# ivclab/CPG

Measured on AMD Instinct MI355X. Metric: images/sec per CPG train-prune-retrain cycle, VGG16 task-1, higher is better.
Workload: dtype f32; 1 GPU; configs[1]: VGG16-BN custom_vgg 224x224, task-1 CPG cycle (finetune -> prune 0.0->0.1 -> recovery, validate after every 20th train step), batch 256 per GPU; task=1, arch=vgg16, global_batch=256, per_gpu_batch=256, parallelism=dp1, epoch_steps=20

## Files before the change

### cpg_amd/csrc/conv3x3_stem.hip

```cpp
#include <algorithm>
#include <type_traits>
#include "cpg_dispatch.h"

using namespace cpg;

namespace {

typedef float f32x2 __attribute__((ext_vector_type(2)));
constexpr int ST_R = 8, ST_W = 32;
constexpr int ST_PW = 36;
constexpr int ST_ROWS = ST_R + 2;
constexpr int ST_CMAX = 3, ST_KS = 14;
constexpr int ST_PATCH = ST_CMAX * ST_ROWS * ST_PW;

struct StemGeom {
    int N, C, K, H, W;
    int tiles_x, tiles_y;
    unsigned ntiles;
};

enum { ST_PLAIN = 0, ST_STATS = 1, ST_STATS_ONLY = 2, ST_BN_RELU = 3, ST_BWD_REDUCE = 4, ST_BWD_APPLY = 5, ST_BWD_WGRAD = 6 };
constexpr int ST_TS = 36;
struct StemBn {
    const float *gamma, *beta, *mean, *invstd;
    const float *coef;
    const float *gz;
};

template <int MODE, int NB = 2, bool RAG = false>
__global__ __launch_bounds__(256, 2)
void k_stem_fwd(StemGeom g, const float *__restrict__ x, const float *__restrict__ w, const float *__restrict__ pm, float thr,
                const float *__restrict__ bias, float *__restrict__ y, float *__restrict__ stats, StemBn bn) {
    constexpr bool STATS = MODE == ST_STATS || MODE == ST_STATS_ONLY || MODE == ST_BWD_REDUCE;
    constexpr bool BN = MODE >= ST_BN_RELU;
    constexpr bool STORE = MODE == ST_PLAIN || MODE == ST_STATS || MODE == ST_BN_RELU || MODE == ST_BWD_APPLY;
    constexpr bool WG = MODE == ST_BWD_WGRAD;
    constexpr bool TWO_PASS = STATS || BN;
    __shared__ float smem_all[4 * ST_PATCH];
    __shared__ __attribute__((aligned(16))) float cst[(MODE >= ST_BWD_REDUCE) ? NB * 32 * 8 : 4];
    const int tid = threadIdx.x, lane = tid & 63, wave = __builtin_amdgcn_readfirstlane(tid >> 6);
    if constexpr (MODE >= ST_BWD_REDUCE) {
        if (tid < NB * 32) {
            const bool kv = tid < g.K;
            cst[tid * 8 + 0] = kv ? bn.mean[tid] : 0.0f, cst[tid * 8 + 1] = kv ? bn.invstd[tid] : 0.0f;
            cst[tid * 8 + 2] = kv ? bn.gamma[tid] : 0.0f, cst[tid * 8 + 3] = kv ? bn.beta[tid] : 0.0f;
            cst[tid * 8 + 4] = (MODE >= ST_BWD_APPLY && kv) ? bn.coef[2 * tid] : 0.0f;
            cst[tid * 8 + 5] = (MODE >= ST_BWD_APPLY && kv) ? bn.coef[2 * tid + 1] : 0.0f;
        }
        __syncthreads();
    }
    const int li = lane & 31, lh = lane >> 5;
    float *smem = smem_all + wave * ST_PATCH;
    const int HW = g.H * g.W, CK = g.C * 9;
    __shared__ __attribute__((aligned(16))) float tsm_all[WG ? 4 * 32 * ST_TS : 4];
    float *tsm = tsm_all + (WG ? wave * 32 * ST_TS : 0);
    const int wk = li < CK ? li : 0, wboff = ((wk / 9) * ST_ROWS + (wk % 9) / 3) * ST_PW + wk % 3 + lh;
    f32x16 accw[WG ? NB : 1];
    if constexpr (WG) {
#pragma unroll
        for (int mb = 0; mb < NB; ++mb)
#pragma unroll
            for (int e = 0; e < 16; ++e) accw[mb][e] = 0.0f;
    }

    constexpr bool ALDS = NB == 3 && TWO_PASS;
    __shared__ float a_lds[ALDS ? NB * ST_KS * 64 : 1];
    float A[ALDS ? 1 : NB][ST_KS];
    int boff[ST_KS];
#pragma unroll
    for (int t = 0; t < ST_KS; ++t) {
        const int k = 2 * t + lh;
        const bool kv = k < CK;
#pragma unroll
        for (int mb = 0; mb < NB; ++mb) {
            const int co = mb * 32 + li;
            float v = 0.0f;
            if (kv && co < g.K) {
                v = w[co * CK + k];
                if (pm != nullptr) v *= binarize(pm[co * CK + k], thr);
            }
            if constexpr (ALDS) {
                if (wave == 0) a_lds[(mb * ST_KS + t) * 64 + lane] = v;
            } else {
                A[mb][t] = v;
            }
        }
        const int kk = kv ? k : 0;
        const int c = kk / 9, r = (kk % 9) / 3, s = kk % 3;
        boff[t] = (c * ST_ROWS + r) * ST_PW + s + li;
    }
    constexpr bool HASB = !BN;
    constexpr bool BPASS = HASB && TWO_PASS && NB == 3;
    float bv[HASB ? (BPASS ? 1 : NB) : 1][HASB ? 16 : 1];
    if constexpr (HASB && !BPASS) {
#pragma unroll
        for (int mb = 0; mb < NB; ++mb)
#pragma unroll
            for (int e = 0; e < 16; ++e) {
                const int co = mb * 32 + (e & 3) + 8 * (e >> 2) + 4 * lh;
                bv[mb][e] = (bias != nullptr && co < g.K) ? bias[co] : 0.0f;
            }
    }

    const __amdgpu_buffer_rsrc_t srd_x = __builtin_amdgcn_make_buffer_rsrc((void *)x, 0, g.N * g.C * HW * 4, 0x00020000);
    constexpr int kOOR = (int)0x80000000;
    const int hw_half = lane >> 5, hcol = lane & 31;
    float pc[15], ph;
    auto tile_coords = [&](unsigned tile, int &n, int &y0, int &x0) {
        const unsigned per_img = (unsigned)(g.tiles_x * g.tiles_y);
        n = (int)(tile / per_img);
        const unsigned r = tile % per_img;
        y0 = (int)(r / (unsigned)g.tiles_x) * ST_R, x0 = (int)(r % (unsigned)g.tiles_x) * ST_W;
    };
    auto issue_loads = [&](unsigned tile) {
        int n, y0, x0;
        tile_coords(tile, n, y0, x0);
#pragma unroll
        for (int q = 0; q < 15; ++q) {
            const int item = 2 * q + hw_half, c = item / ST_ROWS, r = item % ST_ROWS;
            const int row = y0 - 1 + r, col = x0 + hcol;
            const bool ok = c < g.C && (unsigned)row < (unsigned)g.H && col < g.W;
            const int off = ok ? (((n * g.C + c) * g.H + row) * g.W + col) * 4 : kOOR;
            pc[q] = __builtin_bit_cast(float, __builtin_amdgcn_raw_buffer_load_b32(srd_x, off, 0, 0));
        }
        {
            const int item = lane >> 1, side = lane & 1, c = item / ST_ROWS, r = item % ST_ROWS;
            const int row = y0 - 1 + r, col = side ? x0 + ST_W : x0 - 1;
            const bool ok = item < ST_CMAX * ST_ROWS && c < g.C && (unsigned)row < (unsigned)g.H && (unsigned)col < (unsigned)g.W;
            const int off = ok ? (((n * g.C + c) * g.H + row) * g.W + col) * 4 : kOOR;
            ph = __builtin_bit_cast(float, __builtin_amdgcn_raw_buffer_load_b32(srd_x, off, 0, 0));
        }
    };
    auto write_patch = [&]() {
#pragma unroll
        for (int q = 0; q < 15; ++q) smem[(2 * q + hw_half) * ST_PW + 1 + hcol] = pc[q];
        if (lane < 2 * ST_CMAX * ST_ROWS) smem[(lane >> 1) * ST_PW + ((lane & 1) ? ST_W + 1 : 0)] = ph;
    };

    if constexpr (ALDS) __syncthreads();
    const unsigned nwaves = gridDim.x * 4, wid = blockIdx.x * 4 + wave;
    if (wid >= g.ntiles) return;
    const int HW4 = HW * 4;
    issue_loads(wid);
    for (unsigned tile = wid; tile < g.ntiles; tile += nwaves) {
        int n, y0, x0;
        tile_coords(tile, n, y0, x0);
        write_patch();
        if (tile + nwaves < g.ntiles) issue_loads(tile + nwaves);
        float s1[16], s2[16];
        auto zero_sums = [&]() {
            if (STATS) {
#pragma unroll
                for (int e = 0; e < 16; ++e) s1[e] = s2[e] = 0.0f;
            }
        };
        const __amdgpu_buffer_rsrc_t srd_y = __builtin_amdgcn_make_buffer_rsrc((void *)((STORE ? y : (float *)x) + (STORE ? (int64_t)n * g.K * HW : 0)), 0, STORE ? g.K * HW4 : 0, 0x00020000);
        const __amdgpu_buffer_rsrc_t srd_gz = __builtin_amdgcn_make_buffer_rsrc((void *)(MODE >= ST_BWD_REDUCE ? bn.gz + (int64_t)n * g.K * HW : x), 0, MODE >= ST_BWD_REDUCE ? g.K * HW4 : 0, 0x00020000);
        const bool cok = x0 + li < g.W;
        const int pix0 = (y0 * g.W + x0 + li) * 4 + lh * 4 * HW4;
        const bool full = x0 + ST_W <= g.W && y0 + ST_R <= g.H;
        constexpr bool REGC = MODE == ST_BN_RELU;
        float cm[REGC ? 16 : 1], cis[REGC ? 16 : 1], cga[REGC ? 16 : 1], cbe[REGC ? 16 : 1];
        __amdgpu_buffer_rsrc_t srd_bn[4];
        if constexpr (RAG && REGC) {
            srd_bn[0] = __builtin_amdgcn_make_buffer_rsrc((void *)bn.beta, 0, g.K * 4, 0x00020000);
            srd_bn[1] = __builtin_amdgcn_make_buffer_rsrc((void *)bn.mean, 0, g.K * 4, 0x00020000);
            srd_bn[2] = __builtin_amdgcn_make_buffer_rsrc((void *)bn.invstd, 0, g.K * 4, 0x00020000);
            srd_bn[3] = __builtin_amdgcn_make_buffer_rsrc((void *)bn.gamma, 0, g.K * 4, 0x00020000);
        }
        auto load_bn = [&](int mb) {
            if constexpr (BPASS) {
#pragma unroll
                for (int e = 0; e < 16; ++e) {
                    const int co = mb * 32 + (e & 3) + 8 * (e >> 2) + 4 * lh;
                    bv[0][e] = (bias != nullptr && co < g.K) ? bias[co] : 0.0f;
                }
            }
            if constexpr (ALDS) {
#pragma unroll
                for (int t = 0; t < ST_KS; ++t) A[0][t] = a_lds[(mb * ST_KS + t) * 64 + lane];
            }
            if constexpr (REGC) {
#pragma unroll
                for (int e = 0; e < 16; ++e) {
                    if constexpr (RAG) {
                        const int vo = (4 * lh + (e & 3) + 8 * (e >> 2)) * 4 + mb * 128;
                        cm[e] = __builtin_bit_cast(float, __builtin_amdgcn_raw_buffer_load_b32(srd_bn[1], vo, 0, 0));
                        cis[e] = __builtin_bit_cast(float, __builtin_amdgcn_raw_buffer_load_b32(srd_bn[2], vo, 0, 0));
                        cga[e] = __builtin_bit_cast(float, __builtin_amdgcn_raw_buffer_load_b32(srd_bn[3], vo, 0, 0));
                        cbe[e] = __builtin_bit_cast(float, __builtin_amdgcn_raw_buffer_load_b32(srd_bn[0], vo, 0, 0));
                    } else {
                        const int co = mb * 32 + (e & 3) + 8 * (e >> 2) + 4 * lh;
                        cm[e] = bn.mean[co], cis[e] = bn.invstd[co], cga[e] = bn.gamma[co], cbe[e] = bn.beta[co];
                    }
                }
            }
        };
        auto row = [&](int j, auto fullc, auto mbsel) {
            constexpr bool FULL = decltype(fullc)::value;
            constexpr int MB0 = decltype(mbsel)::value < 0 ? 0 : decltype(mbsel)::value, MB1 = decltype(mbsel)::value < 0 ? NB : MB0 + 1;
            const bool pok = FULL || (cok && y0 + j < g.H);
            const int voff = pok ? pix0 + j * g.W * 4 : kOOR;
            int klim = g.K;
            if constexpr (RAG) asm volatile("" : "+s"(klim));
            auto voff_of = [&](int mb, int e) -> int {
                if constexpr (RAG) {
                    if (mb == NB - 1) return ((NB - 1) * 32 + (e & 3) + 8 * (e >> 2) + 4 * lh < klim) ? voff : kOOR;
                }
                return voff;
            };
            float gzv[MODE >= ST_BWD_REDUCE ? 16 : 1];
            int copq = 0;
            if constexpr (MODE >= ST_BWD_REDUCE) asm volatile("" : "+v"(copq));
            if constexpr (MODE >= ST_BWD_REDUCE) {
#pragma unroll
                for (int e = 0; e < 16; ++e)
                    gzv[e] = __builtin_bit_cast(float, __builtin_amdgcn_raw_buffer_load_b32(srd_gz, voff_of(MB0, e), (MB0 * 32 + (e & 3) + 8 * (e >> 2)) * HW4, 0));
            }
            f32x16 acc[NB];
#pragma unroll
            for (int mb = MB0; mb < MB1; ++mb)
#pragma unroll
                for (int e = 0; e < 16; ++e) acc[mb][e] = 0.0f;
            const float *prow = smem + j * ST_PW;
#pragma unroll
            for (int t = 0; t < ST_KS; ++t) {
                const float b = prow[boff[t]];
#pragma unroll
                for (int mb = MB0; mb < MB1; ++mb) acc[mb] = __builtin_amdgcn_mfma_f32_32x32x2f32(A[ALDS ? 0 : mb][t], b, acc[mb], 0, 0, 0);
            }
#pragma unroll
            for (int mb = MB0; mb < MB1; ++mb)
#pragma unroll
                for (int e = 0; e < 16; ++e) {
                    const int cu = mb * 32 + (e & 3) + 8 * (e >> 2);
                    const float v = HASB ? acc[mb][e] + bv[(HASB && !BPASS) ? mb : 0][HASB ? e : 0] : acc[mb][e];
                    if constexpr (MODE == ST_PLAIN || MODE == ST_STATS) {
                        __builtin_amdgcn_raw_buffer_store_b32(__builtin_bit_cast(int, v), srd_y, voff_of(mb, e), cu * HW4, 0);
                    }
                    if constexpr (MODE == ST_STATS || MODE == ST_STATS_ONLY) {
                        const float vm = (FULL || pok) ? v : 0.0f;
                        s1[e] += vm;
                        s2[e] = fmaf(vm, vm, s2[e]);
                    }
                    if constexpr (MODE == ST_BN_RELU) {
                        const float z = relu_keep((v - cm[e]) * cis[e] * cga[e] + cbe[e]);
                        __builtin_amdgcn_raw_buffer_store_b32(__builtin_bit_cast(int, z), srd_y, voff_of(mb, e), cu * HW4, 0);
                    }
                    if constexpr (MODE >= ST_BWD_REDUCE) {
                        const float *cc = cst + (cu + 4 * lh) * 8 + copq;
                        const f32x4 c4 = *reinterpret_cast<const f32x4 *>(cc);
                        const float xh = (v - c4[0]) * c4[1];
                        const float gm = ((v - c4[0]) * c4[1] * c4[2] + c4[3] > 0.0f) ? gzv[e] : 0.0f;
                        if constexpr (MODE == ST_BWD_REDUCE) {
                            s1[e] += gm;
                            s2[e] = fmaf(gm, xh, s2[e]);
                        } else {
                            const f32x2 c2 = *reinterpret_cast<const f32x2 *>(cc + 4);
                            float gyv = (gm - c2[0] - xh * c2[1]) * (c4[1] * c4[2]);
                            if constexpr (MODE == ST_BWD_APPLY) {
                                __builtin_amdgcn_raw_buffer_store_b32(__builtin_bit_cast(int, gyv), srd_y, voff_of(mb, e), cu * HW4, 0);
                            } else {
                                if (!FULL && !pok) gyv = 0.0f;
                                tsm[((e & 3) + 8 * (e >> 2) + 4 * lh) * ST_TS + (li & 1) * 16 + (li >> 1)] = gyv;
                            }
                        }
                    }
                }
            if constexpr (WG) {
                f32x4 ga[4];
#pragma unroll
                for (int q = 0; q < 4; ++q) ga[q] = *reinterpret_cast<const f32x4 *>(tsm + li * ST_TS + lh * 16 + 4 * q);
                const float *brow = smem + j * ST_PW + wboff;
#pragma unroll
                for (int t = 0; t < 16; ++t)
                    accw[MB0] = __builtin_amdgcn_mfma_f32_32x32x2f32(ga[t >> 2][t & 3], brow[2 * t], accw[MB0], 0, 0, 0);
            }
        };
        auto rows = [&](auto mbsel) {
            if (full) {
#pragma unroll 1
                for (int j = 0; j < ST_R; ++j) row(j, std::true_type{}, mbsel);
            } else {
#pragma unroll 1
                for (int j = 0; j < ST_R; ++j) row(j, std::false_type{}, mbsel);
            }
        };
        auto stats_out = [&](int mb) {
#pragma unroll
            for (int e = 0; e < 16; e += 8) half_wave_sum8(s1 + e), half_wave_sum8(s2 + e);
            if (li == kHalfSumLane) {
#pragma unroll
                for (int e = 0; e < 16; ++e) {
                    const int co = mb * 32 + (e & 3) + 8 * (e >> 2) + 4 * lh;
                    if (RAG && co >= g.K) continue;
                    f32x2 o;
                    o[0] = s1[e], o[1] = s2[e];
                    *reinterpret_cast<f32x2 *>(stats + ((int64_t)co * g.ntiles + tile) * 2) = o;
                }
            }
        };
        if (TWO_PASS) {
            load_bn(0);
            zero_sums();
            rows(std::integral_constant<int, 0>{});
            if (STATS) stats_out(0);
            load_bn(1);
            zero_sums();
            rows(std::integral_constant<int, 1>{});
            if (STATS) stats_out(1);
            if constexpr (NB == 3) {
                load_bn(2);
                zero_sums();
                rows(std::integral_constant<int, 2>{});
                if (STATS) stats_out(2);
            }
        } else {
            rows(std::integral_constant<int, -1>{});
        }
    }
    if constexpr (WG) {
        float *dstw = y + (int64_t)wid * g.K * CK;
#pragma unroll
        for (int mb = 0; mb < NB; ++mb)
#pragma unroll
            for (int e = 0; e < 16; ++e) {
                const int co = mb * 32 + (e & 3) + 8 * (e >> 2) + 4 * lh;
                if (li < CK && co < g.K) dstw[co * CK + li] = accw[mb][e];
            }
    }
}

#define STEM_LAUNCH(MODE, grid, block, shm, stream, ...)                                                          \
    do {                                                                                                          \
        if (g.K == 64) hipLaunchKernelGGL((k_stem_fwd<MODE, 2, false>), grid, block, shm, stream, __VA_ARGS__);   \
        else hipLaunchKernelGGL((k_stem_fwd<MODE, 3, true>), grid, block, shm, stream, __VA_ARGS__);              \
    } while (0)

bool stem_geom(int N, int C, int K, int H, int W, StemGeom &g) {
    if (opt_on(OPT_NO_STEM)) return false;
    if (N < 1 || C < 1 || C > ST_CMAX || K < 64 || K > 96 || H < 1 || W < 1) return false;
    if ((int64_t)N * C * H * W * 4 >= (1ll << 31) || (int64_t)K * H * W * 4 >= (1ll << 31)) return false;
    g.N = N, g.C = C, g.K = K, g.H = H, g.W = W;
    g.tiles_x = (W + ST_W - 1) / ST_W, g.tiles_y = (H + ST_R - 1) / ST_R;
    const int64_t nt = (int64_t)N * g.tiles_x * g.tiles_y;
    if (nt >= (1ll << 31)) return false;
    g.ntiles = (unsigned)nt;
    return true;
}

}

extern "C" int cpg_conv3x3_stem_ok(int N, int C, int K, int H, int W) {
    StemGeom g;
    return stem_geom(N, C, K, H, W, g) ? 1 : 0;
}

extern "C" int cpg_conv3x3_stem_tiles(int N, int C, int K, int H, int W) {
    StemGeom g;
    return stem_geom(N, C, K, H, W, g) ? (int)g.ntiles : 0;
}

extern "C" int cpg_conv3x3_stem_run(int N, int C, int K, int H, int W, const float *x, const float *w, const float *pm, float thr,
                                    const float *bias, float *y, float *stats, hipStream_t stream) {
    StemGeom g;
    if (!stem_geom(N, C, K, H, W, g)) return fail(CPG_E_UNSUPPORTED, "cpg_conv2d_fwd(stem): shape not supported");
    unsigned blocks = (unsigned)std::min<int64_t>(((int64_t)g.ntiles + 3) / 4, 4 * kCUs);
    blocks = (unsigned)std::max(1, opt_or(OPT_STEM_BLOCKS, (int)blocks));
    if (stats != nullptr)
        STEM_LAUNCH(ST_STATS, dim3(blocks), dim3(256), 0, stream, g, x, w, pm, thr, bias, y, stats, StemBn{});
    else
        STEM_LAUNCH(ST_PLAIN, dim3(blocks), dim3(256), 0, stream, g, x, w, pm, thr, bias, y, nullptr, StemBn{});
    CPG_CHECK_LAUNCH("cpg_conv2d_fwd(stem)");
    return CPG_OK;
}

namespace {
bool stem_bn_geom(const cpg_conv_desc *d, StemGeom &g) {
    if (opt_on(OPT_NO_STEM_FUSE)) return false;
    if (!(d->R == 3 && d->S == 3 && d->stride_h == 1 && d->stride_w == 1 && d->pad_h == 1 && d->pad_w == 1 && d->dil_h == 1 &&
          d->dil_w == 1 && d->groups == 1))
        return false;
    return stem_geom(d->N, d->C, d->K, d->H, d->W, g);
}
unsigned stem_blocks(const StemGeom &g) {
    unsigned blocks = (unsigned)std::min<int64_t>(((int64_t)g.ntiles + 3) / 4, 4 * kCUs);
    blocks = (unsigned)std::max(1, opt_or(OPT_STEM_BLOCKS, (int)blocks));
    return blocks;
}
}

extern "C" int32_t cpg_stem_bn_supported(const cpg_conv_desc *d) {
    StemGeom g;
    return (d != nullptr && stem_bn_geom(d, g)) ? 1 : 0;
}
extern "C" int32_t cpg_stem_bn_tiles(const cpg_conv_desc *d) {
    StemGeom g;
    return (d != nullptr && stem_bn_geom(d, g)) ? (int32_t)g.ntiles : 0;
}
extern "C" int cpg_stem_bn_stats(const cpg_conv_desc *d, const float *x, const float *w, const float *pm, float thr, const float *bias,
                                 float *stats, size_t stats_bytes, void *stream_v) {
    StemGeom g;
    CPG_REQUIRE(d && x && w && stats, "cpg_stem_bn_stats: null pointer");
    if (!stem_bn_geom(d, g)) return fail(CPG_E_UNSUPPORTED, "cpg_stem_bn_stats: shape not supported");
    if (bias != nullptr) return fail(CPG_E_UNSUPPORTED, "cpg_stem_bn_stats: the fused stem takes no conv bias");
    if (stats_bytes < (size_t)g.K * g.ntiles * 2 * sizeof(float)) return fail(CPG_E_WORKSPACE, "cpg_stem_bn_stats: statistics buffer too small");
    STEM_LAUNCH(ST_STATS_ONLY, dim3(stem_blocks(g)), dim3(256), 0, (hipStream_t)stream_v, g, x, w, pm, thr, bias,
                       (float *)nullptr, stats, StemBn{});
    CPG_CHECK_LAUNCH("cpg_stem_bn_stats");
    return CPG_OK;
}
extern "C" int cpg_stem_bn_relu_fwd(const cpg_conv_desc *d, const float *x, const float *w, const float *pm, float thr, const float *bias,
                                    const float *gamma, const float *beta, const float *mean, const float *invstd, float *z, void *stream_v) {
    StemGeom g;
    CPG_REQUIRE(d && x && w && gamma && beta && mean && invstd && z, "cpg_stem_bn_relu_fwd: null pointer");
    if (!stem_bn_geom(d, g)) return fail(CPG_E_UNSUPPORTED, "cpg_stem_bn_relu_fwd: shape not supported");
    if (bias != nullptr) return fail(CPG_E_UNSUPPORTED, "cpg_stem_bn_relu_fwd: the fused stem takes no conv bias");
    STEM_LAUNCH(ST_BN_RELU, dim3(stem_blocks(g)), dim3(256), 0, (hipStream_t)stream_v, g, x, w, pm, thr, bias, z,
                       (float *)nullptr, StemBn{gamma, beta, mean, invstd, nullptr, nullptr});
    CPG_CHECK_LAUNCH("cpg_stem_bn_relu_fwd");
    return CPG_OK;
}
extern "C" int cpg_stem_bn_relu_bwd_reduce(const cpg_conv_desc *d, const float *x, const float *w, const float *pm, float thr,
                                           const float *bias, const float *gamma, const float *beta, const float *mean, const float *invstd,
                                           const float *gz, float *partials, size_t partials_bytes, void *stream_v) {
    StemGeom g;
    CPG_REQUIRE(d && x && w && gamma && beta && mean && invstd && gz && partials, "cpg_stem_bn_relu_bwd_reduce: null pointer");
    if (!stem_bn_geom(d, g)) return fail(CPG_E_UNSUPPORTED, "cpg_stem_bn_relu_bwd_reduce: shape not supported");
    if (bias != nullptr) return fail(CPG_E_UNSUPPORTED, "cpg_stem_bn_relu_bwd_reduce: the fused stem takes no conv bias");
    if (partials_bytes < (size_t)g.K * g.ntiles * 2 * sizeof(float)) return fail(CPG_E_WORKSPACE, "cpg_stem_bn_relu_bwd_reduce: partial-sum buffer too small");
    STEM_LAUNCH(ST_BWD_REDUCE, dim3(stem_blocks(g)), dim3(256), 0, (hipStream_t)stream_v, g, x, w, pm, thr, bias,
                       (float *)nullptr, partials, StemBn{gamma, beta, mean, invstd, nullptr, gz});
    CPG_CHECK_LAUNCH("cpg_stem_bn_relu_bwd_reduce");
    return CPG_OK;
}
extern "C" int cpg_stem_bn_relu_bwd_apply(const cpg_conv_desc *d, const float *x, const float *w, const float *pm, float thr,
                                          const float *bias, const float *gamma, const float *beta, const float *mean, const float *invstd,
                                          const float *coef, const float *gz, float *gy, void *stream_v) {
    StemGeom g;
    CPG_REQUIRE(d && x && w && gamma && beta && mean && invstd && coef && gz && gy, "cpg_stem_bn_relu_bwd_apply: null pointer");
    if (!stem_bn_geom(d, g)) return fail(CPG_E_UNSUPPORTED, "cpg_stem_bn_relu_bwd_apply: shape not supported");
    if (bias != nullptr) return fail(CPG_E_UNSUPPORTED, "cpg_stem_bn_relu_bwd_apply: the fused stem takes no conv bias");
    STEM_LAUNCH(ST_BWD_APPLY, dim3(stem_blocks(g)), dim3(256), 0, (hipStream_t)stream_v, g, x, w, pm, thr, bias, gy,
                       (float *)nullptr, StemBn{gamma, beta, mean, invstd, coef, gz});
    CPG_CHECK_LAUNCH("cpg_stem_bn_relu_bwd_apply");
    return CPG_OK;
}

extern "C" size_t cpg_stem_bn_wgrad_workspace(const cpg_conv_desc *d) {
    StemGeom g;
    if (d == nullptr || !stem_bn_geom(d, g)) return 0;
    return (size_t)stem_blocks(g) * 4 * g.K * g.C * 9 * sizeof(float);
}
extern "C" int cpg_stem_bn_relu_bwd_wgrad(const cpg_conv_desc *d, const float *x, const float *w, const float *pm, float thr,
                                          const float *bias, const float *gamma, const float *beta, const float *mean, const float *invstd,
                                          const float *coef, const float *gz, float *gw, float *gpm, void *ws, size_t ws_bytes,
                                          void *stream_v) {
    StemGeom g;
    CPG_REQUIRE(d && x && w && gamma && beta && mean && invstd && coef && gz && gw && ws, "cpg_stem_bn_relu_bwd_wgrad: null pointer");
    CPG_REQUIRE((pm == nullptr) == (gpm == nullptr), "cpg_stem_bn_relu_bwd_wgrad: piggymask and its gradient come as a pair");
    if (!stem_bn_geom(d, g)) return fail(CPG_E_UNSUPPORTED, "cpg_stem_bn_relu_bwd_wgrad: shape not supported");
    if (bias != nullptr) return fail(CPG_E_UNSUPPORTED, "cpg_stem_bn_relu_bwd_wgrad: the fused stem takes no conv bias");
    const unsigned blocks = stem_blocks(g);
    if (ws_bytes < (size_t)blocks * 4 * g.K * g.C * 9 * sizeof(float)) return fail(CPG_E_WORKSPACE, "cpg_stem_bn_relu_bwd_wgrad: workspace too small");
    hipStream_t stream = (hipStream_t)stream_v;
    STEM_LAUNCH(ST_BWD_WGRAD, dim3(blocks), dim3(256), 0, stream, g, x, w, pm, thr, bias, (float *)ws, (float *)nullptr,
                       StemBn{gamma, beta, mean, invstd, coef, gz});
    const int nsplit = (int)std::min<int64_t>((int64_t)g.ntiles, (int64_t)blocks * 4);
    Epilogue ep{gw, nullptr, BIAS_NONE, 1, 1, pm, w, gpm, thr};
    launch_split_reduce((const float *)ws, nsplit, (int64_t)g.K * g.C * 9, 0, ep, stream);
    CPG_CHECK_LAUNCH("cpg_stem_bn_relu_bwd_wgrad");
    return CPG_OK;
}
```

### cpg_amd/csrc/cpg_common.cpp

```cpp
#include "cpg_common.h"
#include <stdarg.h>
#include <stdlib.h>
#include <string.h>
#include <atomic>

namespace cpg {

static thread_local char g_err[512] = "";

char *err_buf() { return g_err; }

int fail(int code, const char *fmt, ...) {
    va_list ap;
    va_start(ap, fmt);
    vsnprintf(g_err, sizeof(g_err), fmt, ap);
    va_end(ap);
    return code;
}

static thread_local PackCtx g_pack = {};
PackCtx &pack_ctx() { return g_pack; }
static thread_local WgradRider g_rider = {};
WgradRider &wgrad_rider() { return g_rider; }
static thread_local PoolMaxCtx g_pool_max = {};
PoolMaxCtx &pool_max_ctx() { return g_pool_max; }
static thread_local PoolMaxCtx g_bn_pool_max = {};
PoolMaxCtx &bn_pool_max_ctx() { return g_bn_pool_max; }

int take_packed(size_t bytes, const float **pre, const char *what) {
    PackCtx &c = g_pack;
    *pre = nullptr;
    if (!c.armed) return CPG_OK;
    if (c.use == nullptr || c.use_bytes != bytes || (((uintptr_t)c.use) & 15) != 0)
        return fail(CPG_E_INVALID, "%s: the packed operand handed in (%zu bytes) is not the one this launch streams (%zu bytes, 16-byte aligned)",
                    what, c.use_bytes, bytes);
    *pre = c.use;
    c.armed = false;
    return CPG_OK;
}

static std::atomic<int> g_shared_chip{0};
int shared_chip_hint() { return g_shared_chip.load(std::memory_order_relaxed); }

namespace {
enum Kind { BOOL, INT, WINO_KERNEL };
struct OptDef {
    const char *name;
    Kind kind;
};
const OptDef kDefs[OPT_COUNT] = {
    {"CPG_NO_WINO", BOOL},          {"CPG_NO_WINO_WGRAD", BOOL},   {"CPG_NO_WINO_ODD", BOOL},      {"CPG_NO_STEM", BOOL},
    {"CPG_NO_STEM_FUSE", BOOL},     {"CPG_NO_DEAD_SKIP", BOOL},    {"CPG_NO_S2", BOOL},            {"CPG_NO_V14", BOOL},
    {"CPG_DISABLE_CONV3X3", BOOL},  {"CPG_DISABLE_CONV1X1", BOOL}, {"CPG_DISABLE_CONV1X1_WGRAD", BOOL}, {"CPG_DISABLE_PW_GEMM", BOOL},
    {"CPG_C3_FORCE", INT},          {"CPG_C3W_BPC", INT},          {"CPG_W3_PICK", INT},           {"CPG_PWW_BPC", INT},
    {"CPG_STEM_BLOCKS", INT},       {"CPG_WINO_KERNEL", WINO_KERNEL}, {"CPG_WINO_NW", INT},        {"CPG_WINO_PERSIST", INT},
    {"CPG_WINO_GRIDS", INT},        {"CPG_WW_UNITS", INT},         {"CPG_WW_XCD", INT},            {"CPG_PW_TILE", INT},           {"CPG_WG3_SHARE", INT},
    {"CPG_WW_SHARE", INT},          {"CPG_WINO_TAIL", INT},         {"CPG_FC_SMALL", INT},
    {"CPG_NO_WW_RIDER", BOOL},      {"CPG_NO_GROUPED", BOOL},       {"CPG_GROUPED_WIDE_MIN", INT},
    {"CPG_NO_POOL_MAX", BOOL},
};

struct Table {
    std::atomic<int> v[OPT_COUNT];
    Table() {
        for (int i = 0; i < OPT_COUNT; ++i) {
            int val = OPT_UNSET;
            if (const char *f = getenv(kDefs[i].name)) {
                switch (kDefs[i].kind) {
                    case BOOL: val = (f[0] == 0 || (f[0] == '0' && f[1] == 0)) ? 0 : 1; break;
                    case INT: val = atoi(f); break;
                    case WINO_KERNEL: val = f[0] == 'b' ? 0 : f[0] == 'p' ? 2 : f[0] == '6' ? 3 : 1; break;
                }
            }
            v[i].store(val, std::memory_order_relaxed);
        }
    }
};
Table g_opts;

int find_opt(const char *name) {
    if (name == nullptr) return -1;
    for (int i = 0; i < OPT_COUNT; ++i)
        if (strcmp(name, kDefs[i].name) == 0) return i;
    return -1;
}
}

int opt(Opt o) { return g_opts.v[o].load(std::memory_order_relaxed); }

}

extern "C" int cpg_set_shared_chip_hint(int32_t shared) {
    cpg::g_shared_chip.store(shared ? 1 : 0, std::memory_order_relaxed);
    return CPG_OK;
}
extern "C" int32_t cpg_get_shared_chip_hint(void) { return cpg::shared_chip_hint(); }
extern "C" int cpg_set_option(const char *name, int32_t value) {
    const int i = cpg::find_opt(name);
    if (i < 0) return cpg::fail(CPG_E_INVALID, "cpg_set_option: unknown option '%s'", name ? name : "(null)");
    cpg::g_opts.v[i].store(value, std::memory_order_relaxed);
    return CPG_OK;
}
extern "C" int cpg_get_option(const char *name, int32_t *value) {
    const int i = cpg::find_opt(name);
    if (i < 0 || value == nullptr) return cpg::fail(CPG_E_INVALID, "cpg_get_option: unknown option '%s'", name ? name : "(null)");
    *value = cpg::g_opts.v[i].load(std::memory_order_relaxed);
    return CPG_OK;
}
extern "C" int cpg_version(void) { return CPG_ABI_VERSION; }
extern "C" const char *cpg_last_error(void) { return cpg::err_buf(); }
```

### cpg_amd/csrc/cpg_common.h

```cpp
#pragma once
#include <hip/hip_runtime.h>
#include <stdint.h>
#include <stdio.h>
#include "../../include/cpg_hip.h"

namespace cpg {

char *err_buf();
int fail(int code, const char *fmt, ...);
int shared_chip_hint();

enum Opt {
    OPT_NO_WINO,
    OPT_NO_WINO_WGRAD,
    OPT_NO_WINO_ODD,
    OPT_NO_STEM,
    OPT_NO_STEM_FUSE,
    OPT_NO_DEAD_SKIP,
    OPT_NO_S2,
    OPT_NO_V14,
    OPT_DISABLE_CONV3X3,
    OPT_DISABLE_CONV1X1,
    OPT_DISABLE_CONV1X1_WGRAD,
    OPT_DISABLE_PW_GEMM,
    OPT_C3_FORCE,
    OPT_C3W_BPC,
    OPT_W3_PICK,
    OPT_PWW_BPC,
    OPT_STEM_BLOCKS,
    OPT_WINO_KERNEL,
    OPT_WINO_NW,
    OPT_WINO_PERSIST,
    OPT_WINO_GRIDS,
    OPT_WW_UNITS,
    OPT_WW_XCD,
    OPT_PW_TILE,
    OPT_WG3_SHARE,
    OPT_WW_SHARE,
    OPT_WINO_TAIL,
    OPT_FC_SMALL,
    OPT_NO_WW_RIDER,
    OPT_NO_GROUPED,
    OPT_GROUPED_WIDE_MIN,
    OPT_NO_POOL_MAX,
    OPT_COUNT
};
constexpr int OPT_UNSET = INT32_MIN;
int opt(Opt o);
inline bool opt_on(Opt o) { const int v = opt(o); return v != OPT_UNSET && v != 0; }
inline int opt_or(Opt o, int dflt) { const int v = opt(o); return v == OPT_UNSET ? dflt : v; }

struct PackJob {
    int family;
    int K, C;
    int a, b, c, d;
    long long total;
    size_t bytes;
};
struct PackCtx {
    bool armed;
    const float *use;
    size_t use_bytes;
};
PackCtx &pack_ctx();
int take_packed(size_t bytes, const float **pre, const char *what);
int pack_jobs_launch(const PackJob *ja, float *dst_a, const PackJob *jb, float *dst_b, const float *w, const float *pm, float thr,
                     hipStream_t stream);

struct WgradRider {
    bool armed;
    const float *y, *gz, *table;
    float *gy;
    int N, C, HW;
};
WgradRider &wgrad_rider();

struct PoolMaxCtx {
    bool armed;
    float *E;
    size_t bytes;
};
PoolMaxCtx &pool_max_ctx();
PoolMaxCtx &bn_pool_max_ctx();

inline int hip_status(hipError_t e, const char *what) {
    if (e == hipSuccess) return CPG_OK;
    return fail(CPG_E_HIP_BASE + (int)e, "%s: %s", what, hipGetErrorString(e));
}

#define CPG_CHECK_LAUNCH(what)                                   \
    do {                                                         \
        hipError_t e__ = hipGetLastError();                      \
        if (e__ != hipSuccess) return cpg::hip_status(e__, what); \
    } while (0)

#define CPG_REQUIRE(cond, ...)                                  \
    do {                                                        \
        if (!(cond)) return cpg::fail(CPG_E_INVALID, __VA_ARGS__); \
    } while (0)

__device__ __forceinline__ float binarize(float pm, float thr) {
    return pm > thr ? 1.0f : (pm <= thr ? 0.0f : pm);
}

__device__ __forceinline__ float bn_xhat(float x, float mean, float invstd) { return (x - mean) * invstd; }
__device__ __forceinline__ float bn_affine(float x, float mean, float invstd, float gamma, float beta) {
    return (x - mean) * invstd * gamma + beta;
}
__device__ __forceinline__ float relu_keep(float v) { return v < 0.f ? 0.f : v; }
__device__ __forceinline__ float max_keep(float a, float b) { return __builtin_isunordered(a, b) ? __builtin_nanf("") : fmaxf(a, b); }
__device__ __forceinline__ float bn_relu_affine(float x, float mean, float invstd, float gamma, float beta) {
    return relu_keep(bn_affine(x, mean, invstd, gamma, beta));
}
template <bool RELU, bool TRAIN>
__device__ __forceinline__ float bn_bwd_apply_one(float xv, float gv, float m, float is, float ga, float be, float mg, float mgx, float scale) {
    if (RELU && !(bn_affine(xv, m, is, ga, be) > 0.f)) gv = 0.f;
    return TRAIN ? (gv - mg - bn_xhat(xv, m, is) * mgx) * scale : gv * scale;
}

__device__ __forceinline__ float prelu_one(float v, float a) { return v > 0.f ? v : a * v; }
__device__ __forceinline__ float prelu_sum(float z, float r) {
#pragma clang fp contract(off)
    return z + r;
}
__device__ __forceinline__ float prelu_add(float v, float a, float r) { return prelu_sum(prelu_one(v, a), r); }

constexpr int kCUs = 256;
constexpr int kXCDs = 8;

inline unsigned stream_grid(int64_t work_items, int per_block) {
    int64_t b = (work_items + per_block - 1) / per_block;
    if (b < 1) b = 1;
    if (b > (int64_t)kCUs * 8) b = (int64_t)kCUs * 8;
    return (unsigned)b;
}

typedef float f32x16 __attribute__((ext_vector_type(16)));
typedef float f32x4 __attribute__((ext_vector_type(4)));

}
```

Measured before the change: 2467 images/sec.

## Prefetch stem backward gz rows one row ahead with double buffers

```diff
diff --git a/cpg_amd/csrc/conv3x3_stem.hip b/cpg_amd/csrc/conv3x3_stem.hip
--- a/cpg_amd/csrc/conv3x3_stem.hip
+++ b/cpg_amd/csrc/conv3x3_stem.hip
@@ -27,7 +27,7 @@
     const float *gz;
 };
 
-template <int MODE, int NB = 2, bool RAG = false>
+template <int MODE, int NB = 2, bool RAG = false, bool NEAR = false>
 __global__ __launch_bounds__(256, 2)
 void k_stem_fwd(StemGeom g, const float *__restrict__ x, const float *__restrict__ w, const float *__restrict__ pm, float thr,
                 const float *__restrict__ bias, float *__restrict__ y, float *__restrict__ stats, StemBn bn) {
@@ -36,6 +36,7 @@
     constexpr bool STORE = MODE == ST_PLAIN || MODE == ST_STATS || MODE == ST_BN_RELU || MODE == ST_BWD_APPLY;
     constexpr bool WG = MODE == ST_BWD_WGRAD;
     constexpr bool TWO_PASS = STATS || BN;
+    constexpr bool GZA = (MODE == ST_BWD_REDUCE || MODE == ST_BWD_WGRAD) && !NEAR;
     __shared__ float smem_all[4 * ST_PATCH];
     __shared__ __attribute__((aligned(16))) float cst[(MODE >= ST_BWD_REDUCE) ? NB * 32 * 8 : 4];
     const int tid = threadIdx.x, lane = tid & 63, wave = __builtin_amdgcn_readfirstlane(tid >> 6);
@@ -124,7 +125,9 @@
             pc[q] = __builtin_bit_cast(float, __builtin_amdgcn_raw_buffer_load_b32(srd_x, off, 0, 0));
         }
         {
-            const int item = lane >> 1, side = lane & 1, c = item / ST_ROWS, r = item % ST_ROWS;
+            int hl = lane;
+            if constexpr (GZA) asm volatile("" : "+v"(hl));
+            const int item = hl >> 1, side = hl & 1, c = item / ST_ROWS, r = item % ST_ROWS;
             const int row = y0 - 1 + r, col = side ? x0 + ST_W : x0 - 1;
             const bool ok = item < ST_CMAX * ST_ROWS && c < g.C && (unsigned)row < (unsigned)g.H && (unsigned)col < (unsigned)g.W;
             const int off = ok ? (((n * g.C + c) * g.H + row) * g.W + col) * 4 : kOOR;
@@ -141,12 +144,41 @@
     const unsigned nwaves = gridDim.x * 4, wid = blockIdx.x * 4 + wave;
     if (wid >= g.ntiles) return;
     const int HW4 = HW * 4;
+    float gz0[GZA ? 16 : 1], gz1[GZA ? 16 : 1];
+    auto gz_request = [&](float (&buf)[GZA ? 16 : 1], int n, int yrow, int x0, int mb) {
+        if constexpr (GZA) {
+            __builtin_amdgcn_sched_barrier(0);
+            const __amdgpu_buffer_rsrc_t srd_gz = __builtin_amdgcn_make_buffer_rsrc((void *)(bn.gz + (int64_t)n * g.K * HW), 0, g.K * HW4, 0x00020000);
+            const bool ok = x0 + li < g.W && yrow < g.H;
+            const int voff = ok ? (yrow * g.W + x0 + li) * 4 + lh * 4 * HW4 : kOOR;
+            int klim = g.K;
+            if constexpr (RAG) asm volatile("" : "+s"(klim));
+            const int cleft = klim - mb * 32 - 4 * lh;
+#pragma unroll
+            for (int e = 0; e < 16; ++e) {
+                int off = voff;
+                if constexpr (RAG) off = ((e & 3) + 8 * (e >> 2) < cleft) ? voff : kOOR;
+                buf[e] = __builtin_bit_cast(float, __builtin_amdgcn_raw_buffer_load_b32(srd_gz, off, (mb * 32 + (e & 3) + 8 * (e >> 2)) * HW4, 0));
+            }
+            __builtin_amdgcn_sched_barrier(0);
+        }
+    };
     issue_loads(wid);
+    {
+        int n, y0, x0;
+        tile_coords(wid, n, y0, x0);
+        gz_request(gz0, n, y0, x0, 0);
+    }
     for (unsigned tile = wid; tile < g.ntiles; tile += nwaves) {
         int n, y0, x0;
         tile_coords(tile, n, y0, x0);
         write_patch();
-        if (tile + nwaves < g.ntiles) issue_loads(tile + nwaves);
+        const bool has_next = tile + nwaves < g.ntiles;
+        int nn = n, ny0 = g.H, nx0 = x0;
+        if (has_next) {
+            issue_loads(tile + nwaves);
+            if constexpr (GZA) tile_coords(tile + nwaves, nn, ny0, nx0);
+        }
         float s1[16], s2[16];
         auto zero_sums = [&]() {
             if (STATS) {
@@ -155,7 +187,7 @@
             }
         };
         const __amdgpu_buffer_rsrc_t srd_y = __builtin_amdgcn_make_buffer_rsrc((void *)((STORE ? y : (float *)x) + (STORE ? (int64_t)n * g.K * HW : 0)), 0, STORE ? g.K * HW4 : 0, 0x00020000);
-        const __amdgpu_buffer_rsrc_t srd_gz = __builtin_amdgcn_make_buffer_rsrc((void *)(MODE >= ST_BWD_REDUCE ? bn.gz + (int64_t)n * g.K * HW : x), 0, MODE >= ST_BWD_REDUCE ? g.K * HW4 : 0, 0x00020000);
+        const __amdgpu_buffer_rsrc_t srd_gz = __builtin_amdgcn_make_buffer_rsrc((void *)((MODE >= ST_BWD_REDUCE && !GZA) ? bn.gz + (int64_t)n * g.K * HW : x), 0, (MODE >= ST_BWD_REDUCE && !GZA) ? g.K * HW4 : 0, 0x00020000);
         const bool cok = x0 + li < g.W;
         const int pix0 = (y0 * g.W + x0 + li) * 4 + lh * 4 * HW4;
         const bool full = x0 + ST_W <= g.W && y0 + ST_R <= g.H;
@@ -196,7 +228,7 @@
                 }
             }
         };
-        auto row = [&](int j, auto fullc, auto mbsel) {
+        auto row = [&](int j, auto fullc, auto mbsel, const float (&gza)[GZA ? 16 : 1]) {
             constexpr bool FULL = decltype(fullc)::value;
             constexpr int MB0 = decltype(mbsel)::value < 0 ? 0 : decltype(mbsel)::value, MB1 = decltype(mbsel)::value < 0 ? NB : MB0 + 1;
             const bool pok = FULL || (cok && y0 + j < g.H);
@@ -209,14 +241,15 @@
                 }
                 return voff;
             };
-            float gzv[MODE >= ST_BWD_REDUCE ? 16 : 1];
+            float gzl[(MODE >= ST_BWD_REDUCE && !GZA) ? 16 : 1];
             int copq = 0;
             if constexpr (MODE >= ST_BWD_REDUCE) asm volatile("" : "+v"(copq));
-            if constexpr (MODE >= ST_BWD_REDUCE) {
+            if constexpr (MODE >= ST_BWD_REDUCE && !GZA) {
 #pragma unroll
                 for (int e = 0; e < 16; ++e)
-                    gzv[e] = __builtin_bit_cast(float, __builtin_amdgcn_raw_buffer_load_b32(srd_gz, voff_of(MB0, e), (MB0 * 32 + (e & 3) + 8 * (e >> 2)) * HW4, 0));
-            }
+                    gzl[e] = __builtin_bit_cast(float, __builtin_amdgcn_raw_buffer_load_b32(srd_gz, voff_of(MB0, e), (MB0 * 32 + (e & 3) + 8 * (e >> 2)) * HW4, 0));
+            }
+            const float *gzv = GZA ? gza : gzl;
             f32x16 acc[NB];
 #pragma unroll
             for (int mb = MB0; mb < MB1; ++mb)
@@ -277,18 +310,36 @@
                     accw[MB0] = __builtin_amdgcn_mfma_f32_32x32x2f32(ga[t >> 2][t & 3], brow[2 * t], accw[MB0], 0, 0, 0);
             }
         };
-        auto rows = [&](auto mbsel) {
-            if (full) {
+        auto rows_of = [&](auto fullc, auto mbsel) {
+            if constexpr (GZA) {
+                constexpr int MB = decltype(mbsel)::value;
+                static_assert(ST_R % 2 == 0, "rows in pairs");
 #pragma unroll 1
-                for (int j = 0; j < ST_R; ++j) row(j, std::true_type{}, mbsel);
+                for (int j = 0; j < ST_R; j += 2) {
+                    gz_request(gz1, n, y0 + j + 1, x0, MB);
+                    row(j, fullc, mbsel, gz0);
+                    const bool wrap = j + 2 == ST_R;
+                    if constexpr (MB + 1 < NB) gz_request(gz0, n, wrap ? y0 : y0 + j + 2, x0, wrap ? MB + 1 : MB);
+                    else gz_request(gz0, wrap ? nn : n, wrap ? ny0 : y0 + j + 2, wrap ? nx0 : x0, wrap ? 0 : MB);
+                    row(j + 1, fullc, mbsel, gz1);
+                }
             } else {
 #pragma unroll 1
-                for (int j = 0; j < ST_R; ++j) row(j, std::false_type{}, mbsel);
-            }
+                for (int j = 0; j < ST_R; ++j) row(j, fullc, mbsel, gz0);
+            }
+        };
+        auto rows = [&](auto mbsel) {
+            if (full) rows_of(std::true_type{}, mbsel);
+            else rows_of(std::false_type{}, mbsel);
         };
         auto stats_out = [&](int mb) {
 #pragma unroll
             for (int e = 0; e < 16; e += 8) half_wave_sum8(s1 + e), half_wave_sum8(s2 + e);
+            unsigned ntl = 0;
+            if constexpr (GZA) {
+                ntl = g.ntiles;
+                asm volatile("" : "+s"(ntl));
+            }
             if (li == kHalfSumLane) {
 #pragma unroll
                 for (int e = 0; e < 16; ++e) {
@@ -296,7 +347,7 @@
                     if (RAG && co >= g.K) continue;
                     f32x2 o;
                     o[0] = s1[e], o[1] = s2[e];
-                    *reinterpret_cast<f32x2 *>(stats + ((int64_t)co * g.ntiles + tile) * 2) = o;
+                    *reinterpret_cast<f32x2 *>(stats + ((int64_t)co * (GZA ? ntl : g.ntiles) + tile) * 2) = o;
                 }
             }
         };
@@ -337,6 +388,15 @@
         else hipLaunchKernelGGL((k_stem_fwd<MODE, 3, true>), grid, block, shm, stream, __VA_ARGS__);              \
     } while (0)
 
+#define STEM_LAUNCH_GZ(MODE, grid, block, shm, stream, ...)                                                                   \
+    do {                                                                                                                      \
+        const bool near_ = opt_on(OPT_STEM_GZ_NEAR);                                                                          \
+        if (g.K == 64 && near_) hipLaunchKernelGGL((k_stem_fwd<MODE, 2, false, true>), grid, block, shm, stream, __VA_ARGS__); \
+        else if (g.K == 64) hipLaunchKernelGGL((k_stem_fwd<MODE, 2, false>), grid, block, shm, stream, __VA_ARGS__);          \
+        else if (near_) hipLaunchKernelGGL((k_stem_fwd<MODE, 3, true, true>), grid, block, shm, stream, __VA_ARGS__);         \
+        else hipLaunchKernelGGL((k_stem_fwd<MODE, 3, true>), grid, block, shm, stream, __VA_ARGS__);                          \
+    } while (0)
+
 bool stem_geom(int N, int C, int K, int H, int W, StemGeom &g) {
     if (opt_on(OPT_NO_STEM)) return false;
     if (N < 1 || C < 1 || C > ST_CMAX || K < 64 || K > 96 || H < 1 || W < 1) return false;
@@ -429,8 +489,8 @@
     if (!stem_bn_geom(d, g)) return fail(CPG_E_UNSUPPORTED, "cpg_stem_bn_relu_bwd_reduce: shape not supported");
     if (bias != nullptr) return fail(CPG_E_UNSUPPORTED, "cpg_stem_bn_relu_bwd_reduce: the fused stem takes no conv bias");
     if (partials_bytes < (size_t)g.K * g.ntiles * 2 * sizeof(float)) return fail(CPG_E_WORKSPACE, "cpg_stem_bn_relu_bwd_reduce: partial-sum buffer too small");
-    STEM_LAUNCH(ST_BWD_REDUCE, dim3(stem_blocks(g)), dim3(256), 0, (hipStream_t)stream_v, g, x, w, pm, thr, bias,
-                       (float *)nullptr, partials, StemBn{gamma, beta, mean, invstd, nullptr, gz});
+    STEM_LAUNCH_GZ(ST_BWD_REDUCE, dim3(stem_blocks(g)), dim3(256), 0, (hipStream_t)stream_v, g, x, w, pm, thr, bias,
+                   (float *)nullptr, partials, StemBn{gamma, beta, mean, invstd, nullptr, gz});
     CPG_CHECK_LAUNCH("cpg_stem_bn_relu_bwd_reduce");
     return CPG_OK;
 }
@@ -464,8 +524,8 @@
     const unsigned blocks = stem_blocks(g);
     if (ws_bytes < (size_t)blocks * 4 * g.K * g.C * 9 * sizeof(float)) return fail(CPG_E_WORKSPACE, "cpg_stem_bn_relu_bwd_wgrad: workspace too small");
     hipStream_t stream = (hipStream_t)stream_v;
-    STEM_LAUNCH(ST_BWD_WGRAD, dim3(blocks), dim3(256), 0, stream, g, x, w, pm, thr, bias, (float *)ws, (float *)nullptr,
-                       StemBn{gamma, beta, mean, invstd, coef, gz});
+    STEM_LAUNCH_GZ(ST_BWD_WGRAD, dim3(blocks), dim3(256), 0, stream, g, x, w, pm, thr, bias, (float *)ws, (float *)nullptr,
+                   StemBn{gamma, beta, mean, invstd, coef, gz});
     const int nsplit = (int)std::min<int64_t>((int64_t)g.ntiles, (int64_t)blocks * 4);
     Epilogue ep{gw, nullptr, BIAS_NONE, 1, 1, pm, w, gpm, thr};
     launch_split_reduce((const float *)ws, nsplit, (int64_t)g.K * g.C * 9, 0, ep, stream);
diff --git a/cpg_amd/csrc/cpg_common.cpp b/cpg_amd/csrc/cpg_common.cpp
--- a/cpg_amd/csrc/cpg_common.cpp
+++ b/cpg_amd/csrc/cpg_common.cpp
@@ -57,7 +57,7 @@
     {"CPG_WINO_GRIDS", INT},        {"CPG_WW_UNITS", INT},         {"CPG_WW_XCD", INT},            {"CPG_PW_TILE", INT},           {"CPG_WG3_SHARE", INT},
     {"CPG_WW_SHARE", INT},          {"CPG_WINO_TAIL", INT},         {"CPG_FC_SMALL", INT},
     {"CPG_NO_WW_RIDER", BOOL},      {"CPG_NO_GROUPED", BOOL},       {"CPG_GROUPED_WIDE_MIN", INT},
-    {"CPG_NO_POOL_MAX", BOOL},
+    {"CPG_NO_POOL_MAX", BOOL},      {"CPG_STEM_GZ_NEAR", BOOL},
 };
 
 struct Table {
diff --git a/cpg_amd/csrc/cpg_common.h b/cpg_amd/csrc/cpg_common.h
--- a/cpg_amd/csrc/cpg_common.h
+++ b/cpg_amd/csrc/cpg_common.h
@@ -43,6 +43,7 @@
     OPT_NO_GROUPED,
     OPT_GROUPED_WIDE_MIN,
     OPT_NO_POOL_MAX,
+    OPT_STEM_GZ_NEAR,
     OPT_COUNT
 };
 constexpr int OPT_UNSET = INT32_MIN;
```

Result: no change. 2474 images/sec (median of 6 runs) (+0.3%).
